# Saro00/DGN

Measured on AMD Instinct MI355X. Metric: dgn_layer_fwd_bwd_edges_per_sec, higher is better.
Workload: dtype f32; 1 GPU; c2: ZINC-12k (12000 molecules, one batch), DGN towers: 5 towers, hidden 70, mean max min dir1-av dir1-dx x identity amplification attenuation; edges_per_gpu=586426, nodes_per_gpu=275167, parallelism=single GPU, step=edge weights + layer forward + backward

## Files before the change

dgn_amd/csrc/dgn_abi.hip:

```cpp
#include <hip/hip_runtime.h>

#include <atomic>
#include <cstdarg>
#include <cstdio>
#include <cstdlib>
#include <cstring>
#include <mutex>

#include "dgn_common.hpp"

namespace dgn {
namespace {
thread_local char g_err[512] = "";
}

void set_error(const char* fmt, ...) {
    va_list ap;
    va_start(ap, fmt);
    vsnprintf(g_err, sizeof(g_err), fmt, ap);
    va_end(ap);
}

namespace {
__global__ void zero_rows_kernel(int64_t rows, int64_t width, int64_t ld, float* __restrict__ p) {
// ... 68 lines not shown
    {"tile_gemm", "DGN_TILE_GEMM", -1, false},
    {"tile_wgrad", "DGN_TILE_WGRAD", -1, false},
    {"no_zmask", "DGN_NO_ZMASK", 0, true},
    {"linear_small_min_waves", "DGN_LINEAR_SMALL_MIN_WAVES", 8, false},
    {"graph_bwd_tiles", "DGN_GRAPH_BWD_TILES", 0, false},
    {"odd_direct", "DGN_ODD_DIRECT", 1, false},
    {"bn_from_wgrad", "DGN_BN_FROM_WGRAD", 1, false},
    {"mix_bwd_fused", "DGN_MIX_BWD_FUSED", 1, false},
    {"blk_lds_pad_kb", "DGN_BLK_LDS_PAD_KB", 0, false},
    {"lin_wreg", "DGN_LIN_WREG", 3, false},
    {"bd_bwd_fused", "DGN_BD_BWD_FUSED", 1, false},
    {"bn_stats_fused", "DGN_BN_STATS_FUSED", 1, false},
    {"ew_big_min", "DGN_EW_BIG_MIN", 1 << 19, false},
    {"ew_separate", "DGN_EW_SEPARATE", 0, true},
    {"ew_no_flat8", "DGN_EW_NO_FLAT8", 0, true},
};
std::atomic<int64_t> g_opt[OPT_COUNT];
std::once_flag g_opt_once;
void init_options() {
    for (int i = 0; i < OPT_COUNT; ++i) {
        const char* e = getenv(kOpts[i].env);
        g_opt[i].store(e ? (kOpts[i].presence ? 1 : atoll(e)) : kOpts[i].def, std::memory_order_relaxed);
    }
    if (getenv("DGN_NO_MIX_FUSED")) g_opt[OPT_NO_ZMASK].store(1, std::memory_order_relaxed);
}
int find_option(const char* name) {
    if (name)
        for (int i = 0; i < OPT_COUNT; ++i)
            if (!strcmp(name, kOpts[i].name)) return i;
    return -1;
// ... 32 lines not shown
```

dgn_amd/csrc/dgn_agg.hip:

```cpp
#include <hip/hip_runtime.h>

#include <algorithm>
#include <cstdlib>

#include "dgn_agg_kernels.hpp"

namespace dgn {
namespace {

bool aligned(const void* ptr, int bytes) { return (reinterpret_cast<uintptr_t>(ptr) % bytes) == 0; }

int pick_vec(const DgnAggSpec* spec, const DgnMsg* msg, const float* out, int64_t ld_out, const DgnMsgGrad* gr) {
    const int64_t Ft = msg->F / spec->n_towers;
    for (int vec : {4, 2}) {
        if (msg->f_valid && vec != 2) continue;
        bool ok = (msg->F % vec == 0) && (Ft % vec == 0) && (ld_out % vec == 0) && aligned(out, 4 * vec) && (spec->tower_stride % vec == 0);
        if (msg->F / vec <= 32 && vec > 2) ok = false;
        auto chk = [&](const float* ptr, int64_t ld) {
            if (ptr && (!aligned(ptr, 4 * vec) || ld % vec != 0)) ok = false;
        };
        if (!msg->f_valid) chk(msg->x_src, msg->ld_src);
        chk(msg->x_dst, msg->ld_dst);
        chk(msg->m_edge, msg->ld_edge);
        if (!msg->f_valid) chk(msg->x_in, msg->ld_in);
// ... 314 lines not shown

extern "C" int dgn_agg_backward_aux(const DgnGraph* g, const DgnAggSpec* spec, const DgnMsg* msg, const float* w, int64_t ld_w,
                                    const float* log_deg, const float* g_out, int64_t ld_gout, const unsigned char* aux,
                                    const DgnMsgGrad* grads, void* ws, size_t ws_bytes, void* stream_) {
    if (g && g->n_nodes == 0 && spec && msg && grads) return validate(g, spec, msg, w, log_deg);
    AggParams p;
    float* tab_part = nullptr;
    int rc = agg_backward_prepare(p, g, spec, msg, w, ld_w, log_deg, g_out, ld_gout, false, grads, ws, ws_bytes, stream_, &tab_part, aux);
    if (rc) return rc;
    hipStream_t stream = static_cast<hipStream_t>(stream_);
    const int vec = pick_vec(spec, msg, g_out, ld_gout, grads);
    const unsigned tiles = (unsigned)((msg->F + kWave * vec - 1) / (kWave * vec));
    if (g->blk_cut && g->blk_gap > 0 && g->n_edges > 0 && grads->accumulate == 0 && g->n_hub == 0 && tiles == 1 && vec == 2 && !msg->edge_type &&
        !msg->m_edge && p.g_src && p.x_src && p.n_src == p.n_nodes && !p.g_edge) {
        p.blk_cut = g->blk_cut;
        const int brc = launch_agg_block_v2(p, g->blk_gap, stream);
        if (brc != 1) return brc;
        p.blk_cut = nullptr;
    }
    if (g->gblk_desc && g->n_gblk > 0 && g->csc_order && g->dst_csr && g->csc_ptr && g->n_edges > 0 && grads->accumulate == 0 && g->n_hub == 0 &&
        tiles == 1 && vec == 2 && !msg->edge_type && !msg->m_edge && p.g_src && p.x_src && p.n_src == p.n_nodes && !p.g_edge && !short_rows(p)) {
        p.gblk_desc = g->gblk_desc; p.n_gblk = (int32_t)g->n_gblk; p.gblk_rows = g->gblk_rows; p.csc_order = g->csc_order; p.dst_csr = g->dst_csr;
        p.csc_ptr = g->csc_ptr;
        const int grc = launch_agg_graph_v2(p, stream);
        if (grc != 1) return grc;
        p.gblk_desc = nullptr;
    }
    rc = launch(vec, p, tiles, stream, true);
    if (rc || !msg->edge_type || !grads->g_edge) return rc;
    const int K = msg->n_edge_types, KF = K * (int)msg->F;
    const int waves = std::max(1, std::min(16, 16384 / KF));
    hipLaunchKernelGGL(edge_table_grad_partial, dim3(kTabBlocks), dim3(kWave * waves), (size_t)waves * KF * sizeof(float), stream,
                       p.stage, p.csc_pos, msg->edge_type, p.n_edges, (int)msg->F, K, tab_part);
// ... 6 lines not shown
```

dgn_amd/csrc/dgn_agg_blk_v2.hip:

```cpp
#include "dgn_agg_block.hpp"
#include "dgn_agg_graph.hpp"

namespace dgn {
int launch_agg_block_v2(const AggParams& p, int gap, hipStream_t stream) { return launch_block_vec<2>(p, gap, stream); }
int launch_agg_graph_v2(const AggParams& p, hipStream_t stream) { return launch_graph_v2(p, stream); }
}
```

dgn_amd/csrc/dgn_agg_block.hpp:

```cpp
#pragma once
#include "dgn_agg_kernels.hpp"

namespace dgn {

constexpr int kBlkRowsMax = 56;

template <class C, class O, bool AUX>
__global__ __launch_bounds__(kWave) void agg_bwd_block(const AggParams p0) {
    extern __shared__ float blk_acc[];
    constexpr int VEC = C::VEC, RB = kBwdShortRows;
    static_assert(RB == 4, "groups of four rows");
    const int64_t n_bins = (p0.n_nodes + p0.blk_bin - 1) / p0.blk_bin;
    const int64_t b = xcd_remap(blockIdx.x, n_bins);
    if (b < 0) return;
    const int N = (int)p0.n_nodes;
    const int lo = p0.blk_cut[b * p0.blk_bin];
    const int hi = p0.blk_cut[min((b + 1) * (int64_t)p0.blk_bin, p0.n_nodes)];
    if (lo >= hi) return;
    AggParams p = p0;
    p.blk_lds = blk_acc; p.blk_lo = lo; p.blk_hi = hi;
    const int lo4 = lo & ~(RB - 1), hi4 = min(N, (hi + RB - 1) & ~(RB - 1));
    const int n_ptr = hi4 - lo4 + 1;
    const int ipv_all = p.indptr[lo4 + min(lane_id(), n_ptr - 1)];
    const int n4 = ((hi - lo) * p.F + 3) >> 2;
    for (int i = lane_id(); i < n4; i += kWave) reinterpret_cast<float4*>(blk_acc)[i] = make_float4(0.f, 0.f, 0.f, 0.f);
    const int f0 = lane_id() * VEC;
    const bool active = f0 < p.F;
    auto ptr_at = [&](int i) { return bcast_i(ipv_all, min(i, n_ptr - 1)); };
    constexpr bool AHEAD = n_gout_blocks<O>() <= 2;
    SlotBatch<C::NCH, C::NW> cur, nxt;
    GroupRows<C, RB, n_gout_blocks<O>(), AUX> rows, rows_nxt;
    cur.load_raw(p, ptr_at(0));
    if constexpr (AHEAD) load_group_rows<C, O, RB, AUX>(rows, p, lo4, f0);
    for (int row0 = lo4; row0 < hi; row0 += RB) {
        const int off = row0 - lo4;
        nxt.load_raw(p, ptr_at(off + RB));
        if constexpr (AHEAD) load_group_rows<C, O, RB, AUX>(rows_nxt, p, row0 + RB, f0);
        const int nrows = min(RB, N - row0);
        const int ipv = __shfl(ipv_all, min(off + min(lane_id(), RB), n_ptr - 1), kWave);
        bwd_short_group<C, O, RB, false, false, AUX, true, AHEAD>(p, row0, nrows, f0, active, ipv, &cur, &rows);
        cur = nxt;
        if constexpr (AHEAD) rows = rows_nxt;
    }
    if (active) {
        for (int r = 0; r < hi - lo; ++r) {
            float v[VEC];
            ldv<VEC>(v, blk_acc + r * p.F + f0);
            stv<VEC>(p.g_src + (int64_t)(lo + r) * p.ldg_src + f0, v);
        }
// ... 7 lines not shown
    const int bin = rcap - gap + 1;
    if (bin < 4) return false;
    out.bin = bin; out.rows = rcap;
    out.lds = (((size_t)rcap * F * 4) + 15) & ~(size_t)15;
    return true;
}

template <class C, class O>
int launch_backward_block_cfg(const AggParams& p, int gap, hipStream_t stream) {
    BlkPlan plan;
    if (p.n_nodes < option(OPT_BLK_MIN_NODES) || !short_rows(p) || option(OPT_BWD_ROWS_PER_WAVE) <= 1 || !blk_plan(plan, p.F, gap)) return 1;
    AggParams q = p;
    q.stage = nullptr; q.csc_pos = nullptr; q.csc_ptr = nullptr; q.fresh = true; q.seg_add = false;
    q.blk_bin = plan.bin; q.blk_rows = plan.rows;
    const int64_t n_bins = (p.n_nodes + plan.bin - 1) / plan.bin;
    const dim3 grid((unsigned)xcd_grid(n_bins)), block(kWave);
    plan.lds += (size_t)std::max<int64_t>(0, option(OPT_BLK_LDS_PAD_KB)) * 1024;
    if constexpr (C::NCH <= 2) {
        if (p.aux) {
            hipLaunchKernelGGL((agg_bwd_block<C, O, true>), grid, block, plan.lds, stream, q);
            DGN_HIP_CHECK(hipGetLastError());
            return DGN_OK;
        }
    }
    hipLaunchKernelGGL((agg_bwd_block<C, O, false>), grid, block, plan.lds, stream, q);
    DGN_HIP_CHECK(hipGetLastError());
    return DGN_OK;
}

template <int VEC>
int launch_block_vec(const AggParams& p, int gap, hipStream_t stream) {
// ... 12 lines not shown
```

dgn_amd/csrc/dgn_agg_kernels.hpp:

```cpp
#pragma once
#include <hip/hip_runtime.h>

#include <cmath>
#include <cstdlib>

#include "dgn_common.hpp"

#ifndef DGN_UNROLL
#define DGN_UNROLL 8
#endif

namespace dgn {

enum : uint32_t {
    NEED_SQ = 2u, NEED_MAX = 4u, NEED_MIN = 8u,
    NEED_XIN = 16u,
    NEED_RECOMP = 32u,
    NEED_M_EMIT = 64u,
    NEED_XPASS = 128u
};

struct AggParams {
    const int32_t* indptr;
    const int32_t* src;
// ... 43 lines not shown
    float* part_sw;
    float* coef;
    float* stage;
    unsigned char* aux;
    int32_t aux_rows;
    int32_t stage_out;
    bool fresh;
    bool seg_add;
    const int32_t* csc_ptr;
    const int32_t* csc_pos;
    int32_t n_slots;
    int32_t n_coef;
    const int32_t* blk_cut;
    int32_t blk_bin;
    int32_t blk_rows;
    const int32_t* gblk_desc; const int32_t* csc_order; const int32_t* dst_csr;
    int32_t n_gblk, gblk_rows;
    float* blk_lds;
    int32_t blk_lo, blk_hi;
};

inline void pack_agg_list(AggParams& p, const DgnAggSpec* spec) {
    p.op_pack = p.ch_pack = 0; p.any_av = false;
    uint32_t need = 0;
    for (int a = 0; a < spec->n_agg; ++a) {
        const int op = spec->agg_op[a], c = spec->agg_ch[a];
        p.op_pack |= (uint64_t)op << (4 * a);
        p.ch_pack |= (uint64_t)((op >= DGN_AGG_DIR_AV && op <= DGN_AGG_DIR_DX_NO_ABS) ? c : 0) << (3 * a);
        switch (op) {
            case DGN_AGG_MAX: need |= NEED_MAX | NEED_RECOMP; break;
// ... 1940 lines not shown
```

dgn_amd/csrc/dgn_common.hpp:

```cpp
#pragma once
#include <hip/hip_runtime.h>
#include <stdint.h>

#include <atomic>

#include "dgn_hip.h"

namespace dgn {

constexpr int kWave = 64;
#ifndef DGN_WAVES_PER_BLOCK
#define DGN_WAVES_PER_BLOCK 1
#endif
constexpr int kWavesPerBlock = DGN_WAVES_PER_BLOCK;
constexpr int kBlock = kWave * kWavesPerBlock;
constexpr int kXcds = 8;

void set_error(const char* fmt, ...);
enum Opt { OPT_BLK_LDS_KB, OPT_BLK_MIN_NODES, OPT_BWD_ROWS_PER_WAVE, OPT_TILE_GEMM, OPT_TILE_WGRAD, OPT_NO_ZMASK, OPT_LINEAR_SMALL_MIN_WAVES, OPT_GRAPH_BWD_TILES, OPT_ODD_DIRECT, OPT_BN_FROM_WGRAD, OPT_MIX_BWD_FUSED, OPT_BLK_LDS_PAD_KB, OPT_LIN_WREG, OPT_BD_BWD_FUSED, OPT_BN_STATS_FUSED, OPT_EW_BIG_MIN, OPT_EW_SEPARATE, OPT_EW_NO_FLAT8, OPT_COUNT };
int64_t option(Opt o);
int hip_fail(hipError_t e, const char* what);
int zero_rows_async(float* p, int64_t rows, int64_t width, int64_t ld, hipStream_t stream);
int scale_rows_async(int64_t n_rows, int32_t width, const float* g, int64_t ld_g, const float* g_loss, float* out, int64_t ld_out, hipStream_t stream);

using LdsOptIn = std::atomic<unsigned long long>;
hipError_t allow_lds(LdsOptIn& done, int bytes, const void* const* kernels, int n_kernels);
template <class... K>
inline hipError_t allow_lds(LdsOptIn& done, int bytes, K*... kernels) {
    const void* const list[] = {reinterpret_cast<const void*>(kernels)...};
    return allow_lds(done, bytes, list, (int)sizeof...(K));
}
int n_cus();
inline bool al16(const void* q) { return (reinterpret_cast<uintptr_t>(q) & 15) == 0; }

// ... 55 lines not shown
__device__ __forceinline__ float bcast_f(float v, int lane) {
    return __int_as_float(__builtin_amdgcn_readlane(__float_as_int(v), lane));
}
__device__ __forceinline__ int uniform_i(int v) { return __builtin_amdgcn_readfirstlane(v); }

__device__ __forceinline__ int64_t xcd_remap(int64_t b, int64_t n_logical) {
#ifdef DGN_EXP_NOREMAP
    return b < n_logical ? b : -1;
#endif
    int64_t per = (n_logical + kXcds - 1) / kXcds;
    int64_t logical = (b % kXcds) * per + b / kXcds;
    return logical < n_logical ? logical : -1;
}
inline int64_t xcd_grid(int64_t n_logical) { return ((n_logical + kXcds - 1) / kXcds) * kXcds; }

template <int VEC>
__device__ __forceinline__ void ldv(float (&d)[VEC], const float* p) {
    if constexpr (VEC == 4) {
        float4 t = *reinterpret_cast<const float4*>(p);
        d[0] = t.x; d[1] = t.y; d[2] = t.z; d[3] = t.w;
    } else if constexpr (VEC == 2) {
        float2 t = *reinterpret_cast<const float2*>(p);
        d[0] = t.x; d[1] = t.y;
    } else {
        d[0] = *p;
    }
}
template <int VEC>
__device__ __forceinline__ void stv(float* p, const float (&d)[VEC]) {
    if constexpr (VEC == 4) {
// ... 86 lines not shown
```

dgn_amd/csrc/dgn_graph_build.hip:

```cpp
#include <hip/hip_runtime.h>
#include <hipcub/hipcub.hpp>

#include <cmath>
#include <cstdint>

#include "dgn_common.hpp"

namespace dgn {
namespace {

inline size_t up256(size_t x) { return (x + 255) & ~(size_t)255; }
inline unsigned blocks(int64_t n, int per = 256) { return (unsigned)((n + per - 1) / per); }
inline int bits_for(int64_t n) { int b = 1; while (((int64_t)1 << b) < n && b < 31) ++b; return b; }

__global__ void gb_prepare(int64_t E, const int64_t* __restrict__ dst, int32_t* __restrict__ key, int32_t* __restrict__ val,
                           int32_t* __restrict__ deg) {
    const int64_t e = (int64_t)blockIdx.x * blockDim.x + threadIdx.x;
    if (e >= E) return;
    const int d = (int)dst[e];
    key[e] = d;
    val[e] = (int)e;
    atomicAdd(deg + d, 1);
}
__global__ void gb_gather(int64_t E, const int64_t* __restrict__ src, const int32_t* __restrict__ perm, int32_t* __restrict__ src_csr,
// ... 39 lines not shown
        atomicAdd(diff + a + 1, 1);
        atomicAdd(diff + b + 1, -1);
    }
}
__global__ void gb_mark_closed(int64_t N, const int32_t* __restrict__ cross, int32_t* __restrict__ val) {
    const int64_t i = (int64_t)blockIdx.x * blockDim.x + threadIdx.x;
    if (i <= N) val[i] = cross[i] == 0 ? (int)i : 0;
}
__global__ void gb_max_gap(int64_t N, const int32_t* __restrict__ cross, const int32_t* __restrict__ lastcut, int32_t* __restrict__ gap_out) {
    const int64_t i = (int64_t)blockIdx.x * blockDim.x + threadIdx.x + 1;
    int g = 0;
    if (i <= N && cross[i] == 0) g = (int)i - lastcut[i - 1];
#pragma unroll
    for (int o = 32; o > 0; o >>= 1) g = max(g, __shfl_xor(g, o, kWave));
    if ((threadIdx.x & 63) == 0 && g > 0) atomicMax(gap_out, g);
}

size_t cub_bytes(int64_t n) {
    size_t a = 0, b = 0;
    int32_t* p = nullptr;
    hipcub::DeviceRadixSort::SortPairs(nullptr, a, p, p, p, p, (int)n);
    hipcub::DeviceScan::ExclusiveSum(nullptr, b, p, p, (int)n);
    size_t c = 0;
    hipcub::DeviceScan::InclusiveScan(nullptr, c, p, p, hipcub::Max(), (int)n);
    return up256(std::max(std::max(a, b), c)) + 256;
}

}
}

// ... 49 lines not shown
    int32_t* cross = reinterpret_cast<int32_t*>(w); w += nbytes;
    int32_t* val = reinterpret_cast<int32_t*>(w); w += nbytes;
    void* cub = w;
    size_t cub_sz = ws_bytes - (size_t)(w - static_cast<char*>(ws));
    DGN_HIP_CHECK(hipMemsetAsync(diff, 0, (size_t)(n_nodes + 2) * 4, st));
    DGN_HIP_CHECK(hipMemsetAsync(gap_out, 0, sizeof(int32_t), st));
    if (n_edges > 0) hipLaunchKernelGGL(gb_span, dim3(blocks(n_edges)), dim3(256), 0, st, n_edges, src_csr, dst_csr, diff);
    DGN_HIP_CHECK(hipcub::DeviceScan::InclusiveSum(cub, cub_sz, diff, cross, (int)(n_nodes + 1), st));
    hipLaunchKernelGGL(gb_mark_closed, dim3(blocks(n_nodes + 1)), dim3(256), 0, st, n_nodes, cross, val);
    DGN_HIP_CHECK(hipcub::DeviceScan::InclusiveScan(cub, cub_sz, val, blk_cut, hipcub::Max(), (int)(n_nodes + 1), st));
    if (n_nodes > 0) hipLaunchKernelGGL(gb_max_gap, dim3(blocks(n_nodes)), dim3(256), 0, st, n_nodes, cross, blk_cut, gap_out);
    DGN_HIP_CHECK(hipGetLastError());
    return DGN_OK;
}

extern "C" int dgn_graph_build_csc(int64_t n_nodes, int64_t n_edges, const int32_t* src_csr, int32_t* csc_ptr, int32_t* csc_pos,
                                   int32_t* csc_order, void* ws, size_t ws_bytes, void* stream_) {
    const char* fn = "dgn_graph_build_csc";
    if (!csc_ptr || (n_edges > 0 && (!src_csr || !csc_pos || !csc_order))) { set_error("%s: null array", fn); return DGN_ERR_INVALID; }
    if (!ws || ws_bytes < dgn_graph_build_workspace_bytes(n_nodes, n_edges)) { set_error("%s: workspace too small", fn); return DGN_ERR_WORKSPACE; }
    hipStream_t st = static_cast<hipStream_t>(stream_);
    char* w = static_cast<char*>(ws);
    const size_t eb = up256((size_t)(n_edges + 1) * 4), nbytes = up256((size_t)(n_nodes + 2) * 4);
    int32_t* val = reinterpret_cast<int32_t*>(w); w += eb;
    int32_t* key_out = reinterpret_cast<int32_t*>(w); w += eb;
    w += 2 * eb;
    int32_t* hist = reinterpret_cast<int32_t*>(w); w += nbytes;
    w += 3 * nbytes;
    w += up256((size_t)n_edges + 1);
    void* cub = w;
// ... 12 lines not shown
```

dgn_amd/graph.py:

```python
from __future__ import annotations

import ctypes as C
import os
from typing import Dict, Optional, Tuple

import functools

import torch

from . import _lib
from .spec import EPS, AggPlan, Channel

HUB_THRESHOLD = 2048
HUB_CHUNK = 1024
NATIVE_BUILD = True
DC_CLASSES, DC_UNIT = _lib.DGN_DC_CLASSES, _lib.DGN_DC_UNIT
GRAPH_BLOCK_MAX_ROWS = 512
BLOCK_MAX_GAP = 52
DEFERRED_STATS = True


def _ptr(t: Optional[torch.Tensor]) -> Optional[int]:
    return None if t is None else t.data_ptr()

# ... 141 lines not shown
                ent["overflow_event"].record(torch.cuda.current_stream(self.device))
                ent["overflow_pending"] = True
                self._check_block_overflow(ent)
        if not getattr(self, "_stats_pending", False):
            return
        self._stats_event.synchronize()
        self._stats_pending = False
        max_deg, n_hub = int(self._stats_host[0]), int(self._stats_host[1])
        self.max_in_degree = max_deg
        if n_hub:
            raise _lib.DgnError("padded graphs take batches without hub rows (in-degree <= hub_threshold) only "
                                f"(the batch loaded before this call had {n_hub}, largest in-degree {max_deg})")

    def invalidate_caches(self) -> None:
        self._wcache.clear()
        for k in ("_scale_cache", "_dst_slots", "_eig_norm", "_slot_types", "_dc", "_dc_split", "_dc_scale", "_blk", "_blk_tables"):
            self.__dict__.pop(k, None)
        if hasattr(self, "_c"):
            self._c.blk_cut, self._c.blk_gap = None, 0
            self._c.gblk_desc, self._c.n_gblk, self._c.gblk_rows, self._c.dst_csr = None, 0, 0, None

    def _build_native(self, src, dst, num_nodes, hub_threshold, hub_chunk):
        lib = _lib.load()
        dev, E = src.device, src.numel()
        if num_nodes >= 2 ** 31 - 1 or E >= 2 ** 31 - 1:
            raise ValueError("graph exceeds the int32 CSR range")
        src64, dst64 = src.long().contiguous(), dst.long().contiguous()
        i32 = lambda n: torch.empty(n, dtype=torch.int32, device=dev)
        indptr, src_csr, dst_csr = i32(num_nodes + 1), i32(E), i32(E)
        eid = torch.empty(E, dtype=torch.int64, device=dev)
        log_deg = torch.empty(num_nodes, dtype=torch.float32, device=dev)
        deg = torch.empty(num_nodes, dtype=torch.int64, device=dev)
        stats = i32(4)
        nbytes = lib.dgn_graph_build_workspace_bytes(num_nodes, E)
# ... 133 lines not shown
        self.csc_ptr, self.csc_pos, order = i32(N + 1), i32(E), i32(E)
        self.csc_order = order
        _lib.check(lib.dgn_graph_build_csc(N, E, self.src.data_ptr(), self.csc_ptr.data_ptr(), self.csc_pos.data_ptr(), order.data_ptr(),
                                           ws.data_ptr(), nbytes, stream), "dgn_graph_build_csc")
        self._c.csc_ptr, self._c.csc_pos = self.csc_ptr.data_ptr(), self.csc_pos.data_ptr()

    def _closed_cuts(self):
        if "_blk" not in self.__dict__:
            lib = _lib.load()
            N, E, dev = self.num_nodes, self.num_edges, self.device
            dst_csr = getattr(self, "dst_csr", None)
            if dst_csr is None:
                deg = (self.indptr[1:] - self.indptr[:-1]).long()
                dst_csr = torch.repeat_interleave(torch.arange(N, device=dev, dtype=torch.int32), deg)
                self.dst_csr = dst_csr
            cut = torch.empty(N + 1, dtype=torch.int32, device=dev)
            gap = torch.zeros(1, dtype=torch.int32, device=dev)
            nbytes = lib.dgn_graph_build_workspace_bytes(N, E)
            ws = torch.empty(nbytes, dtype=torch.uint8, device=dev)
            _lib.check(lib.dgn_graph_build_cuts(N, E, self.src.data_ptr(), dst_csr.data_ptr(), cut.data_ptr(), gap.data_ptr(),
                                                ws.data_ptr(), nbytes, _lib.stream_ptr(dev)), "dgn_graph_build_cuts")
            self._blk = (cut, int(gap.item()))
        return self._blk

    def block_table(self, graph_sizes=None, target_rows=None):
        if getattr(self, "_pad", None) is not None:
            return self.__dict__.get("_blk_static") if target_rows is None else None
        tables = self.__dict__.setdefault("_blk_tables", {})
        ent = tables.get(target_rows)
        if ent is not None:
            return ent or None
        if not (self.src.is_cuda and self.num_src == self.num_nodes and self.n_hub == 0 and getattr(self, "_pad", None) is None
                and self.row_base == 0 and self.num_edges > 0 and self.num_nodes > 0):
            tables[target_rows] = {}
            return None
        if torch.cuda.is_current_stream_capturing():
            return None
        import numpy as np
# ... 65 lines not shown
        ent["desc"].copy_(ent["host"], non_blocking=True)
        ent["copied"].record(torch.cuda.current_stream(self.device))
        ent["overflow_host"].copy_(ent["overflow"], non_blocking=True)
        ent["overflow_event"].record(torch.cuda.current_stream(self.device))
        ent["overflow_pending"] = True

    def _check_block_overflow(self, ent) -> None:
        if ent.get("overflow_pending"):
            ent["overflow_event"].synchronize()
            ent["overflow_pending"] = False
            if int(ent["overflow_host"][0]):
                ent["overflow"].zero_()
                raise _lib.DgnError(f"a batch held a graph beyond the block capacity ({ent['max_rows']} rows / {ent['max_edges']} edges): its rows "
                                    "were skipped by the graph-block layer kernels (set_block_capacity with larger bounds)")

    def ensure_blocks(self, enabled: bool = True) -> bool:
        ok = False
        min_nodes = int(_lib.options.blk_min_nodes)
        if enabled and self.src.is_cuda and self.num_src == self.num_nodes and self.n_hub == 0 and getattr(self, "_pad", None) is None \
                and self.num_nodes >= max(1, min_nodes) and 0 < self.num_edges <= 3 * self.num_nodes and self.row_base == 0:
            if "_blk" not in self.__dict__ and torch.cuda.is_current_stream_capturing():
                enabled = False
            if enabled and "_blk" not in self.__dict__:
                self._closed_cuts()
            if enabled:
                cut, gap = self._blk
                ok = 0 < gap <= BLOCK_MAX_GAP
        if ok:
            self._c.blk_cut, self._c.blk_gap = cut.data_ptr(), gap
        else:
            self._c.blk_cut, self._c.blk_gap = None, 0
        self._ensure_graph_blocks(enabled)
        return ok

    def _ensure_graph_blocks(self, enabled: bool = True) -> bool:
        ok = False
        if enabled and self.src.is_cuda and self.num_src == self.num_nodes and self.n_hub == 0 and getattr(self, "_pad", None) is None \
                and self.row_base == 0 and self.num_edges > 3 * self.num_nodes:
            t = self.block_table(target_rows=1)
            if t is not None and t["max_rows"] <= GRAPH_BLOCK_MAX_ROWS and getattr(self, "_csc_ready", False) and hasattr(self, "csc_order"):
                self._closed_cuts()
                self._c.gblk_desc, self._c.n_gblk, self._c.gblk_rows = t["desc"].data_ptr(), t["n_blocks"], t["max_rows"]
                self._c.csc_order, self._c.dst_csr = self.csc_order.data_ptr(), self.dst_csr.data_ptr()
                ok = True
        if not ok:
            self._c.gblk_desc, self._c.n_gblk, self._c.gblk_rows, self._c.csc_order, self._c.dst_csr = None, 0, 0, None, None
# ... 93 lines not shown
```

dgn_amd/ops.py:

```python
from __future__ import annotations

import ctypes as C
import os
from typing import Optional

import torch

from . import _lib
from .graph import DGNGraph, _ptr
from .spec import EPS, AggPlan


DETERMINISTIC_BACKWARD = "auto"


def _two_phase_scatter(F: int) -> bool:
    return (F % 2 == 0) if DETERMINISTIC_BACKWARD == "auto" else bool(DETERMINISTIC_BACKWARD)


BLOCK_BACKWARD = os.environ.get("DGN_BLOCK_BACKWARD", "1") != "0"

_N_VALID = None


# ... 121 lines not shown
    grads.g_src, grads.ld_src = _ptr(g_src), _ld(g_src)
    grads.g_dst, grads.ld_dst = _ptr(g_dst), _ld(g_dst)
    grads.g_edge, grads.ld_edge = _ptr(g_edge), _ld(g_edge)
    grads.g_in, grads.ld_in = _ptr(g_in), _ld(g_in)
    msg = _msg_struct(F, x_src, x_dst, m_edge, x_in, edge_type, f_valid)
    stream = _lib.stream_ptr(dev)
    tower_stride, ld_gout = _out_layout(g_out)
    specs = _spec_structs(plan, n_towers, avg_log, tower_stride)
    g = graph.c_graph
    first = True
    deterministic = _two_phase_scatter(F) and g_src is not None
    if edge_type is not None and not deterministic:
        raise _lib.DgnError("edge-type table: the backward needs the two-phase scatter (even F, a gradient for x_src)")
    if deterministic:
        graph.ensure_csc()
    graph.ensure_blocks(bool(BLOCK_BACKWARD) and deterministic and not accumulate and len(plan.launches) == 1)
    for spec, l in zip(specs, plan.launches):
        nbytes = lib.dgn_agg_backward_workspace_bytes(C.byref(g), C.byref(spec), F, 1 if deterministic else 0)
        if edge_type is not None:
            nbytes += lib.dgn_agg_edge_table_workspace_bytes(F, m_edge.shape[0])
        ws = torch.empty(nbytes, dtype=torch.uint8, device=dev) if nbytes else None
        wl = w[l.ch_offset:] if (w is not None and l.channels) else None
        tmp = None
        if g_edge is not None and not first:
            tmp = torch.empty_like(g_edge)
            grads.g_edge = tmp.data_ptr()
        grads.accumulate = 1 if (accumulate or not first) else 0
        rc = lib.dgn_agg_backward_aux(C.byref(g), C.byref(spec), C.byref(msg), _ptr(wl), w.stride(0) if w is not None else 0,
                                      graph.log_deg.data_ptr(), g_out.data_ptr(), ld_gout, _ptr(aux), C.byref(grads),
                                      _ptr(ws), nbytes, stream)
        _lib.check(rc, "dgn_agg_backward")
# ... 804 lines not shown
        return out

    @staticmethod
    def backward(ctx, g_out):
        lib = _lib.load()
        w_edge, h, snorm, scale, w_sd, bias_sd, w_post, b_post, gamma, beta, w_mix, b_mix, saved_buf, aux, drop_mask = ctx.saved_tensors
        graph, plan, cfg = ctx.graph, ctx.plan, ctx.cfg
        T, fi, fo, S = cfg[:4]
        id_slot = cfg[9] if len(cfg) > 9 else None
        N, Fm, Fo = h.shape[0], T * fi, T * fo
        K = plan.n_agg * fi
        dev = h.device
        _, bufs = _carve(_towers_saved_sizes(cfg, plan, N, ctx.n_y1, ctx.n_z), dev, saved_buf)
        g_out = g_out.contiguous()
        graph.ensure_csc()
        graph.ensure_blocks(bool(BLOCK_BACKWARD))
        L, keep = _towers_struct(graph, plan, ctx.avg_log, w_edge, cfg, h, snorm, scale, w_sd, bias_sd, w_post, b_post, gamma, beta, w_mix, b_mix, bufs,
                                 ctx.use_mask, aux, drop_mask, ctx.n_valid)
        L.id_slot1 = 0 if id_slot is None else int(id_slot) + 1
        ws = _layer_workspace(L, lib.dgn_towers_layer_backward_workspace_bytes(C.byref(L)), dev)
        g_h = torch.empty((N, Fm), dtype=torch.float32, device=dev)
        n_ops = [2 * Fm * Fm, 2 * Fm, Fo, Fo, Fo, T * S * fo * K]
        n_flat = _up64(sum(n_ops))
        gbuf = torch.empty(n_flat + _up64(Fo * Fo) + Fo, dtype=torch.float32, device=dev)
        g_w_sd, g_bias_sd, g_b_post, g_gamma, g_beta, g_w_post = gbuf[:sum(n_ops)].split(n_ops)
        g_w_mix, g_b_mix = gbuf[n_flat:n_flat + Fo * Fo], gbuf[n_flat + _up64(Fo * Fo):]
        G = _lib.DgnTowersGrads(g_out=g_out.data_ptr(), g_h=g_h.data_ptr(), g_w_sd=g_w_sd.data_ptr(), g_bias_sd=g_bias_sd.data_ptr(),
                                g_w_post=g_w_post.data_ptr(), g_b_post=g_b_post.data_ptr(), g_gamma=g_gamma.data_ptr(),
                                g_beta=g_beta.data_ptr(), g_w_mix=g_w_mix.data_ptr(), g_b_mix=g_b_mix.data_ptr())
        _lib.check(lib.dgn_towers_layer_backward(C.byref(L), C.byref(G), _lib.stream_ptr(dev)), "dgn_towers_layer_backward")
        return (None, None, None, None, None, g_h, None, None, None, None, None, g_w_sd.view(2 * Fm, Fm), g_bias_sd, g_w_post.view(T, S * fo, K),
# ... 242 lines not shown
        ctx.save_for_backward(w_edge, h, snorm, scale, w_pre, b_pre, w_post, b_post, gamma, beta, saved_buf, aux)
        ctx.graph, ctx.plan, ctx.avg_log, ctx.cfg = graph, plan, avg_log, cfg
        return out

    @staticmethod
    def backward(ctx, g_out):
        lib = _lib.load()
        w_edge, h, snorm, scale, w_pre, b_pre, w_post, b_post, gamma, beta, saved_buf, aux = ctx.saved_tensors
        cfg, graph = ctx.cfg, ctx.graph
        type_net, F0, fo = cfg[:3]
        N, dev = h.shape[0], h.device
        sizes, Fp, K = _dense_sizes(cfg, N, ctx.dc is not None)
        _, bufs = _carve_ptrs(sizes, dev, saved_buf)
        g_out = g_out.contiguous()
        graph.ensure_csc()
        graph.ensure_blocks(bool(BLOCK_BACKWARD))
        L, keep = _dense_struct(graph, ctx.plan, ctx.avg_log, w_edge, cfg, h, snorm, scale, w_pre, b_pre, w_post, b_post, gamma, beta, bufs, ctx.n_valid,
                                ctx.dc)
        L.agg_aux = _ptr(aux)
        ws = _layer_workspace(L, lib.dgn_dense_layer_backward_workspace_bytes(C.byref(L)), dev)
        g_h = torch.empty((N, F0), dtype=torch.float32, device=dev)
        n_pre = w_pre.numel() if w_pre is not None else 0
        _, (g_w_pre, g_b_pre, g_w_post, g_b_post, g_gamma, g_beta) = _carve([n_pre, F0 if (type_net == 1 and b_pre is not None) else 0, w_post.numel(), fo, fo, fo], dev)
        q = lambda t: t.data_ptr() if t.numel() else None
        G = _lib.DgnDenseGrads(g_out=g_out.data_ptr(), g_h=g_h.data_ptr(), g_w_pre=q(g_w_pre), g_b_pre=q(g_b_pre), g_w_post=g_w_post.data_ptr(),
                               g_b_post=g_b_post.data_ptr(), g_gamma=g_gamma.data_ptr(), g_beta=g_beta.data_ptr())
        stream = _lib.stream_ptr(dev)
        _lib.check(lib.dgn_dense_layer_backward(C.byref(L), C.byref(G), stream), "dgn_dense_layer_backward")
        return (None, None, None, None, None, g_h, None, None, None, None, None,
                g_w_pre.view_as(w_pre) if w_pre is not None else None, g_b_pre if (b_pre is not None and type_net == 1) else None,
                g_w_post.view_as(w_post), g_b_post if b_post is not None else None, g_gamma, g_beta)
# ... 786 lines not shown
```

include/dgn_hip.h:

```cpp
#ifndef DGN_HIP_H
#define DGN_HIP_H

#include <stddef.h>
#include <stdint.h>

#ifdef __cplusplus
extern "C" {
#endif

#define DGN_ABI_VERSION 38

#define DGN_MAX_AGG 16
#define DGN_MAX_CH 4
#define DGN_MAX_SCALERS 4

enum {
    DGN_OK = 0,
    DGN_ERR_INVALID = -1,
    DGN_ERR_WORKSPACE = -2,
    DGN_ERR_HIP = -3
};

enum {
    DGN_AGG_MEAN = 0,
    DGN_AGG_SUM = 1,
// ... 27 lines not shown
    const int32_t* src;
    int64_t n_hub;
    const int32_t* hub_rows;
    const int32_t* hub_chunk_ptr;
    int64_t n_chunks;
    const int32_t* chunk_hub;
    int32_t hub_threshold;
    int32_t hub_chunk;
    const int32_t* csc_ptr;
    const int32_t* csc_pos;
    int32_t max_in_degree;
    int64_t n_src;
    int64_t row_base;
    const int32_t* blk_cut;
    int32_t blk_gap;
    const int32_t* gblk_desc; int64_t n_gblk; int32_t gblk_rows;
    const int32_t* csc_order;
    const int32_t* dst_csr;
} DgnGraph;

typedef struct DgnChannel {
    int32_t kind;
    int32_t eig_col;
    float alpha;
    float eps;
} DgnChannel;

typedef struct DgnAggSpec {
    int32_t n_agg;
    int32_t agg_op[DGN_MAX_AGG];
// ... 163 lines not shown
                   int64_t lddw, float* dbias, void* ws, size_t ws_bytes, void* stream);

int dgn_layer_fused_supported(const DgnGraph* g, const DgnAggSpec* spec, int64_t F, int32_t n_scalers, int32_t f_out);
int dgn_layer_fused_forward(const DgnGraph* g, const DgnAggSpec* spec, const DgnMsg* msg, const float* w, int64_t ld_w,
                            const float* log_deg, const float* weight, int64_t ldw, int64_t stride_w, int32_t n_scalers,
                            int32_t f_out, const float* scale, const float* bias, const float* row_scale, float* y, int64_t ld_y,
                            void* stream);
size_t dgn_graph_build_workspace_bytes(int64_t n_nodes, int64_t n_edges);
int dgn_graph_build(int64_t n_nodes, int64_t n_edges, const int64_t* src, const int64_t* dst, int32_t* indptr, int32_t* src_csr,
                    int32_t* dst_csr, int64_t* eid, float* log_deg, int64_t* in_degree, int32_t* stats, int32_t hub_threshold,
                    void* ws, size_t ws_bytes, void* stream);
int dgn_graph_build_cuts(int64_t n_nodes, int64_t n_edges, const int32_t* src_csr, const int32_t* dst_csr, int32_t* blk_cut,
                         int32_t* gap_out, void* ws, size_t ws_bytes, void* stream);
int dgn_graph_build_csc(int64_t n_nodes, int64_t n_edges, const int32_t* src_csr, int32_t* csc_ptr, int32_t* csc_pos,
                        int32_t* csc_order, void* ws, size_t ws_bytes, void* stream);


typedef struct DgnTowersLayer {
    const DgnGraph* graph;
    const DgnAggSpec* spec;
    const float* w;
    int64_t ld_w;
    const float* log_deg;
    int32_t n_towers, f_in, f_out, n_scalers;
    int32_t residual;
    float momentum, eps, slope;
    const float* h;
    const float* snorm;
    const float* scale;
    const float* w_sd;  const float* bias_sd;
// ... 281 lines not shown
```

Baseline: 506.8 million edges/s.

## Schedule block-backward bins from a precomputed, work-sorted task list

Adds a per-graph task list of int4 records (row range, starting edge pointer, group count), built once after the block cuts, and sorts the bins by descending work so heavy bins launch first. The block backward kernel reads its task from this list instead of the XCD remap and cut lookups, and in the EARLY case it preloads the first group's rows and the next slot batch before entering the main loop. The intent is to reduce tail imbalance and startup latency per block. In exchange it adds a one-time radix sort and task build stored past the end of the cut array, drops the XCD-aware block mapping, and has extra logic for graph-capture caching.

```diff
diff --git a/dgn_amd/csrc/dgn_abi.hip b/dgn_amd/csrc/dgn_abi.hip
--- a/dgn_amd/csrc/dgn_abi.hip
+++ b/dgn_amd/csrc/dgn_abi.hip
@@ -106,6 +106,7 @@
     {"ew_big_min", "DGN_EW_BIG_MIN", 1 << 19, false},
     {"ew_separate", "DGN_EW_SEPARATE", 0, true},
     {"ew_no_flat8", "DGN_EW_NO_FLAT8", 0, true},
+    {"blk_task_list", "DGN_BLK_TASK_LIST", 2, false},
 };
 std::atomic<int64_t> g_opt[OPT_COUNT];
 std::once_flag g_opt_once;
diff --git a/dgn_amd/csrc/dgn_agg.hip b/dgn_amd/csrc/dgn_agg.hip
--- a/dgn_amd/csrc/dgn_agg.hip
+++ b/dgn_amd/csrc/dgn_agg.hip
@@ -352,9 +352,13 @@
     if (g->blk_cut && g->blk_gap > 0 && g->n_edges > 0 && grads->accumulate == 0 && g->n_hub == 0 && tiles == 1 && vec == 2 && !msg->edge_type &&
         !msg->m_edge && p.g_src && p.x_src && p.n_src == p.n_nodes && !p.g_edge) {
         p.blk_cut = g->blk_cut;
+        if (g->blk_task_bin > 0) {
+            p.blk_task = reinterpret_cast<const int4*>(g->blk_cut + blk_task_offset(g->n_nodes));
+            p.blk_task_bin = g->blk_task_bin;
+        }
         const int brc = launch_agg_block_v2(p, g->blk_gap, stream);
         if (brc != 1) return brc;
-        p.blk_cut = nullptr;
+        p.blk_cut = nullptr; p.blk_task = nullptr; p.blk_task_bin = 0;
     }
     if (g->gblk_desc && g->n_gblk > 0 && g->csc_order && g->dst_csr && g->csc_ptr && g->n_edges > 0 && grads->accumulate == 0 && g->n_hub == 0 &&
         tiles == 1 && vec == 2 && !msg->edge_type && !msg->m_edge && p.g_src && p.x_src && p.n_src == p.n_nodes && !p.g_edge && !short_rows(p)) {
diff --git a/dgn_amd/csrc/dgn_agg_blk_v2.hip b/dgn_amd/csrc/dgn_agg_blk_v2.hip
--- a/dgn_amd/csrc/dgn_agg_blk_v2.hip
+++ b/dgn_amd/csrc/dgn_agg_blk_v2.hip
@@ -5,3 +5,11 @@
 int launch_agg_block_v2(const AggParams& p, int gap, hipStream_t stream) { return launch_block_vec<2>(p, gap, stream); }
 int launch_agg_graph_v2(const AggParams& p, hipStream_t stream) { return launch_graph_v2(p, stream); }
 }
+
+extern "C" int dgn_agg_block_plan(int64_t F, int32_t gap, int32_t* bin, int32_t* rows) {
+    dgn::BlkPlan plan;
+    if (F <= 0 || gap <= 0 || !dgn::blk_plan(plan, F, gap)) return 1;
+    if (bin) *bin = plan.bin;
+    if (rows) *rows = plan.rows;
+    return 0;
+}
diff --git a/dgn_amd/csrc/dgn_agg_block.hpp b/dgn_amd/csrc/dgn_agg_block.hpp
--- a/dgn_amd/csrc/dgn_agg_block.hpp
+++ b/dgn_amd/csrc/dgn_agg_block.hpp
@@ -11,11 +11,19 @@
     constexpr int VEC = C::VEC, RB = kBwdShortRows;
     static_assert(RB == 4, "groups of four rows");
     const int64_t n_bins = (p0.n_nodes + p0.blk_bin - 1) / p0.blk_bin;
-    const int64_t b = xcd_remap(blockIdx.x, n_bins);
-    if (b < 0) return;
     const int N = (int)p0.n_nodes;
-    const int lo = p0.blk_cut[b * p0.blk_bin];
-    const int hi = p0.blk_cut[min((b + 1) * (int64_t)p0.blk_bin, p0.n_nodes)];
+    const bool listed = p0.blk_task != nullptr;
+    int lo, hi, ptr0 = 0;
+    if (listed) {
+        if ((int64_t)blockIdx.x >= n_bins) return;
+        const int4 t = p0.blk_task[blockIdx.x];
+        lo = t.x; hi = t.y; ptr0 = t.z;
+    } else {
+        const int64_t b = xcd_remap(blockIdx.x, n_bins);
+        if (b < 0) return;
+        lo = p0.blk_cut[b * p0.blk_bin];
+        hi = p0.blk_cut[min((b + 1) * (int64_t)p0.blk_bin, p0.n_nodes)];
+    }
     if (lo >= hi) return;
     AggParams p = p0;
     p.blk_lds = blk_acc; p.blk_lo = lo; p.blk_hi = hi;
@@ -30,9 +38,20 @@
     constexpr bool AHEAD = n_gout_blocks<O>() <= 2;
     SlotBatch<C::NCH, C::NW> cur, nxt;
     GroupRows<C, RB, n_gout_blocks<O>(), AUX> rows, rows_nxt;
-    cur.load_raw(p, ptr_at(0));
-    if constexpr (AHEAD) load_group_rows<C, O, RB, AUX>(rows, p, lo4, f0);
-    for (int row0 = lo4; row0 < hi; row0 += RB) {
+    constexpr bool EARLY = !AHEAD && (n_gout_blocks<O>() <= 4 || (n_gout_blocks<O>() == 5 && AUX));
+    cur.load_raw(p, listed ? ptr0 : ptr_at(0));
+    if (AHEAD || (EARLY && listed)) load_group_rows<C, O, RB, AUX>(rows, p, lo4, f0);
+    int row0 = lo4;
+    if constexpr (EARLY) {
+        if (listed) {
+            nxt.load_raw(p, ptr_at(RB));
+            const int ipv = __shfl(ipv_all, min(min(lane_id(), RB), n_ptr - 1), kWave);
+            bwd_short_group<C, O, RB, false, false, AUX, true, true>(p, row0, min(RB, N - row0), f0, active, ipv, &cur, &rows);
+            cur = nxt;
+            row0 += RB;
+        }
+    }
+    for (; row0 < hi; row0 += RB) {
         const int off = row0 - lo4;
         nxt.load_raw(p, ptr_at(off + RB));
         if constexpr (AHEAD) load_group_rows<C, O, RB, AUX>(rows_nxt, p, row0 + RB, f0);
@@ -70,7 +89,8 @@
     q.stage = nullptr; q.csc_pos = nullptr; q.csc_ptr = nullptr; q.fresh = true; q.seg_add = false;
     q.blk_bin = plan.bin; q.blk_rows = plan.rows;
     const int64_t n_bins = (p.n_nodes + plan.bin - 1) / plan.bin;
-    const dim3 grid((unsigned)xcd_grid(n_bins)), block(kWave);
+    if (p.blk_task_bin != plan.bin || option(OPT_BLK_TASK_LIST) == 0) q.blk_task = nullptr;
+    const dim3 grid((unsigned)(q.blk_task ? n_bins : xcd_grid(n_bins))), block(kWave);
     plan.lds += (size_t)std::max<int64_t>(0, option(OPT_BLK_LDS_PAD_KB)) * 1024;
     if constexpr (C::NCH <= 2) {
         if (p.aux) {
diff --git a/dgn_amd/csrc/dgn_agg_kernels.hpp b/dgn_amd/csrc/dgn_agg_kernels.hpp
--- a/dgn_amd/csrc/dgn_agg_kernels.hpp
+++ b/dgn_amd/csrc/dgn_agg_kernels.hpp
@@ -81,6 +81,8 @@
     const int32_t* blk_cut;
     int32_t blk_bin;
     int32_t blk_rows;
+    const int4* blk_task;
+    int32_t blk_task_bin;
     const int32_t* gblk_desc; const int32_t* csc_order; const int32_t* dst_csr;
     int32_t n_gblk, gblk_rows;
     float* blk_lds;
diff --git a/dgn_amd/csrc/dgn_common.hpp b/dgn_amd/csrc/dgn_common.hpp
--- a/dgn_amd/csrc/dgn_common.hpp
+++ b/dgn_amd/csrc/dgn_common.hpp
@@ -17,7 +17,7 @@
 constexpr int kXcds = 8;
 
 void set_error(const char* fmt, ...);
-enum Opt { OPT_BLK_LDS_KB, OPT_BLK_MIN_NODES, OPT_BWD_ROWS_PER_WAVE, OPT_TILE_GEMM, OPT_TILE_WGRAD, OPT_NO_ZMASK, OPT_LINEAR_SMALL_MIN_WAVES, OPT_GRAPH_BWD_TILES, OPT_ODD_DIRECT, OPT_BN_FROM_WGRAD, OPT_MIX_BWD_FUSED, OPT_BLK_LDS_PAD_KB, OPT_LIN_WREG, OPT_BD_BWD_FUSED, OPT_BN_STATS_FUSED, OPT_EW_BIG_MIN, OPT_EW_SEPARATE, OPT_EW_NO_FLAT8, OPT_COUNT };
+enum Opt { OPT_BLK_LDS_KB, OPT_BLK_MIN_NODES, OPT_BWD_ROWS_PER_WAVE, OPT_TILE_GEMM, OPT_TILE_WGRAD, OPT_NO_ZMASK, OPT_LINEAR_SMALL_MIN_WAVES, OPT_GRAPH_BWD_TILES, OPT_ODD_DIRECT, OPT_BN_FROM_WGRAD, OPT_MIX_BWD_FUSED, OPT_BLK_LDS_PAD_KB, OPT_LIN_WREG, OPT_BD_BWD_FUSED, OPT_BN_STATS_FUSED, OPT_EW_BIG_MIN, OPT_EW_SEPARATE, OPT_EW_NO_FLAT8, OPT_BLK_TASK_LIST, OPT_COUNT };
 int64_t option(Opt o);
 int hip_fail(hipError_t e, const char* what);
 int zero_rows_async(float* p, int64_t rows, int64_t width, int64_t ld, hipStream_t stream);
@@ -103,6 +103,8 @@
 }
 inline int64_t xcd_grid(int64_t n_logical) { return ((n_logical + kXcds - 1) / kXcds) * kXcds; }
 
+inline int64_t blk_task_offset(int64_t n_nodes) { return (n_nodes + 4) & ~(int64_t)3; }
+
 template <int VEC>
 __device__ __forceinline__ void ldv(float (&d)[VEC], const float* p) {
     if constexpr (VEC == 4) {
diff --git a/dgn_amd/csrc/dgn_graph_build.hip b/dgn_amd/csrc/dgn_graph_build.hip
--- a/dgn_amd/csrc/dgn_graph_build.hip
+++ b/dgn_amd/csrc/dgn_graph_build.hip
@@ -77,6 +77,31 @@
 #pragma unroll
     for (int o = 32; o > 0; o >>= 1) g = max(g, __shfl_xor(g, o, kWave));
     if ((threadIdx.x & 63) == 0 && g > 0) atomicMax(gap_out, g);
+}
+
+__device__ __forceinline__ int4 gb_task_of(int64_t b, int64_t N, int bin, const int32_t* __restrict__ cut, const int32_t* __restrict__ indptr) {
+    const int lo = cut[b * bin], hi = cut[min((b + 1) * (int64_t)bin, N)];
+    if (lo >= hi) return make_int4(lo, hi, indptr[lo & ~3], 0);
+    return make_int4(lo, hi, indptr[lo & ~3], (hi - (lo & ~3) + 3) >> 2);
+}
+constexpr int kTaskKeyBits = 5;
+__global__ void gb_task_keys(int64_t n_bins, int64_t N, int bin, const int32_t* __restrict__ cut, const int32_t* __restrict__ indptr,
+                             int32_t* __restrict__ key, int32_t* __restrict__ val) {
+    const int64_t b = (int64_t)blockIdx.x * blockDim.x + threadIdx.x;
+    if (b >= n_bins) return;
+    key[b] = min(gb_task_of(b, N, bin, cut, indptr).w, (1 << kTaskKeyBits) - 1);
+    val[b] = (int)b;
+}
+__global__ void gb_task_records(int64_t n_bins, int64_t N, int bin, const int32_t* __restrict__ cut, const int32_t* __restrict__ indptr,
+                                const int32_t* __restrict__ order, int4* __restrict__ tasks) {
+    const int64_t i = (int64_t)blockIdx.x * blockDim.x + threadIdx.x;
+    if (i < n_bins) tasks[i] = gb_task_of(order ? order[i] : i, N, bin, cut, indptr);
+}
+size_t task_sort_bytes(int64_t n) {
+    size_t a = 0;
+    int32_t* p = nullptr;
+    hipcub::DeviceRadixSort::SortPairsDescending(nullptr, a, p, p, p, p, (int)n, 0, kTaskKeyBits);
+    return up256(a) + 256;
 }
 
 size_t cub_bytes(int64_t n) {
@@ -156,6 +181,46 @@
     return DGN_OK;
 }
 
+extern "C" int64_t dgn_blk_cut_capacity(int64_t n_nodes) {
+    return n_nodes < 0 ? 0 : blk_task_offset(n_nodes) + 4 * ((n_nodes + 3) / 4);
+}
+
+extern "C" size_t dgn_graph_build_tasks_workspace_bytes(int64_t n_nodes, int32_t bin) {
+    if (n_nodes < 0 || bin < 4) return 0;
+    const int64_t n_bins = (n_nodes + bin - 1) / bin;
+    return 4 * up256((size_t)(n_bins + 1) * 4) + task_sort_bytes(n_bins + 1);
+}
+
+extern "C" int dgn_graph_build_tasks(int64_t n_nodes, const int32_t* indptr, int32_t* blk_cut, int32_t bin, void* ws, size_t ws_bytes,
+                                     void* stream_) {
+    const char* fn = "dgn_graph_build_tasks";
+    if (n_nodes < 0 || n_nodes >= INT32_MAX - 1) { set_error("%s: sizes outside the int32 CSR range", fn); return DGN_ERR_INVALID; }
+    if (bin < 4) { set_error("%s: a bin has at least 4 rows", fn); return DGN_ERR_INVALID; }
+    if (!blk_cut || !indptr) { set_error("%s: null array", fn); return DGN_ERR_INVALID; }
+    if (reinterpret_cast<uintptr_t>(blk_cut) & 15) { set_error("%s: blk_cut is not 16-byte aligned", fn); return DGN_ERR_INVALID; }
+    if (!ws || ws_bytes < dgn_graph_build_tasks_workspace_bytes(n_nodes, bin)) { set_error("%s: workspace too small", fn); return DGN_ERR_WORKSPACE; }
+    if (n_nodes == 0) return DGN_OK;
+    hipStream_t st = static_cast<hipStream_t>(stream_);
+    const int64_t n_bins = (n_nodes + bin - 1) / bin;
+    int4* tasks = reinterpret_cast<int4*>(blk_cut + blk_task_offset(n_nodes));
+    const int32_t* order = nullptr;
+    if (option(OPT_BLK_TASK_LIST) != 1) {
+        char* w = static_cast<char*>(ws);
+        const size_t kb = up256((size_t)(n_bins + 1) * 4);
+        int32_t* key = reinterpret_cast<int32_t*>(w); w += kb;
+        int32_t* key_out = reinterpret_cast<int32_t*>(w); w += kb;
+        int32_t* val = reinterpret_cast<int32_t*>(w); w += kb;
+        int32_t* val_out = reinterpret_cast<int32_t*>(w); w += kb;
+        size_t cub_sz = ws_bytes - (size_t)(w - static_cast<char*>(ws));
+        hipLaunchKernelGGL(gb_task_keys, dim3(blocks(n_bins)), dim3(256), 0, st, n_bins, n_nodes, (int)bin, (const int32_t*)blk_cut, indptr, key, val);
+        DGN_HIP_CHECK(hipcub::DeviceRadixSort::SortPairsDescending(w, cub_sz, key, key_out, val, val_out, (int)n_bins, 0, kTaskKeyBits, st));
+        order = val_out;
+    }
+    hipLaunchKernelGGL(gb_task_records, dim3(blocks(n_bins)), dim3(256), 0, st, n_bins, n_nodes, (int)bin, (const int32_t*)blk_cut, indptr, order, tasks);
+    DGN_HIP_CHECK(hipGetLastError());
+    return DGN_OK;
+}
+
 extern "C" int dgn_graph_build_csc(int64_t n_nodes, int64_t n_edges, const int32_t* src_csr, int32_t* csc_ptr, int32_t* csc_pos,
                                    int32_t* csc_order, void* ws, size_t ws_bytes, void* stream_) {
     const char* fn = "dgn_graph_build_csc";
diff --git a/dgn_amd/graph.py b/dgn_amd/graph.py
--- a/dgn_amd/graph.py
+++ b/dgn_amd/graph.py
@@ -179,10 +179,10 @@
 
     def invalidate_caches(self) -> None:
         self._wcache.clear()
-        for k in ("_scale_cache", "_dst_slots", "_eig_norm", "_slot_types", "_dc", "_dc_split", "_dc_scale", "_blk", "_blk_tables"):
+        for k in ("_scale_cache", "_dst_slots", "_eig_norm", "_slot_types", "_dc", "_dc_split", "_dc_scale", "_blk", "_blk_tasks", "_blk_tasks_captured", "_blk_tables"):
             self.__dict__.pop(k, None)
         if hasattr(self, "_c"):
-            self._c.blk_cut, self._c.blk_gap = None, 0
+            self._c.blk_cut, self._c.blk_gap, self._c.blk_task_bin = None, 0, 0
             self._c.gblk_desc, self._c.n_gblk, self._c.gblk_rows, self._c.dst_csr = None, 0, 0, None
 
     def _build_native(self, src, dst, num_nodes, hub_threshold, hub_chunk):
@@ -346,14 +346,39 @@
                 deg = (self.indptr[1:] - self.indptr[:-1]).long()
                 dst_csr = torch.repeat_interleave(torch.arange(N, device=dev, dtype=torch.int32), deg)
                 self.dst_csr = dst_csr
-            cut = torch.empty(N + 1, dtype=torch.int32, device=dev)
+            cut = torch.empty(lib.dgn_blk_cut_capacity(N), dtype=torch.int32, device=dev)[:N + 1]
             gap = torch.zeros(1, dtype=torch.int32, device=dev)
             nbytes = lib.dgn_graph_build_workspace_bytes(N, E)
             ws = torch.empty(nbytes, dtype=torch.uint8, device=dev)
             _lib.check(lib.dgn_graph_build_cuts(N, E, self.src.data_ptr(), dst_csr.data_ptr(), cut.data_ptr(), gap.data_ptr(),
                                                 ws.data_ptr(), nbytes, _lib.stream_ptr(dev)), "dgn_graph_build_cuts")
             self._blk = (cut, int(gap.item()))
+            self.__dict__.pop("_blk_tasks", None)
+            self.__dict__.pop("_blk_tasks_captured", None)
         return self._blk
+
+    def _block_tasks(self, width: int) -> int:
+        lib = _lib.load()
+        mode = int(_lib.options.blk_task_list)
+        cut, gap = self._blk
+        bin_ = C.c_int32(0)
+        if mode == 0 or lib.dgn_agg_block_plan(int(width), gap, C.byref(bin_), None) != 0:
+            return 0
+        key = (bin_.value, mode)
+        capturing = torch.cuda.is_current_stream_capturing()
+        if self.__dict__.get("_blk_tasks") != key:
+            if capturing or self.__dict__.get("_blk_tasks_captured"):
+                return 0
+            N, dev = self.num_nodes, self.device
+            nbytes = lib.dgn_graph_build_tasks_workspace_bytes(N, bin_.value)
+            ws = torch.empty(nbytes, dtype=torch.uint8, device=dev)
+            self.__dict__.pop("_blk_tasks", None)
+            _lib.check(lib.dgn_graph_build_tasks(N, self.indptr.data_ptr(), cut.data_ptr(), bin_.value, ws.data_ptr(), nbytes,
+                                                 _lib.stream_ptr(dev)), "dgn_graph_build_tasks")
+            self._blk_tasks = key
+        if capturing:
+            self._blk_tasks_captured = True
+        return bin_.value
 
     def block_table(self, graph_sizes=None, target_rows=None):
         if getattr(self, "_pad", None) is not None:
@@ -449,7 +474,7 @@
                 raise _lib.DgnError(f"a batch held a graph beyond the block capacity ({ent['max_rows']} rows / {ent['max_edges']} edges): its rows "
                                     "were skipped by the graph-block layer kernels (set_block_capacity with larger bounds)")
 
-    def ensure_blocks(self, enabled: bool = True) -> bool:
+    def ensure_blocks(self, enabled: bool = True, width: int = 0) -> bool:
         ok = False
         min_nodes = int(_lib.options.blk_min_nodes)
         if enabled and self.src.is_cuda and self.num_src == self.num_nodes and self.n_hub == 0 and getattr(self, "_pad", None) is None \
@@ -463,8 +488,9 @@
                 ok = 0 < gap <= BLOCK_MAX_GAP
         if ok:
             self._c.blk_cut, self._c.blk_gap = cut.data_ptr(), gap
+            self._c.blk_task_bin = self._block_tasks(width) if width > 0 else 0
         else:
-            self._c.blk_cut, self._c.blk_gap = None, 0
+            self._c.blk_cut, self._c.blk_gap, self._c.blk_task_bin = None, 0, 0
         self._ensure_graph_blocks(enabled)
         return ok
 
diff --git a/dgn_amd/ops.py b/dgn_amd/ops.py
--- a/dgn_amd/ops.py
+++ b/dgn_amd/ops.py
@@ -159,7 +159,7 @@
         raise _lib.DgnError("edge-type table: the backward needs the two-phase scatter (even F, a gradient for x_src)")
     if deterministic:
         graph.ensure_csc()
-    graph.ensure_blocks(bool(BLOCK_BACKWARD) and deterministic and not accumulate and len(plan.launches) == 1)
+    graph.ensure_blocks(bool(BLOCK_BACKWARD) and deterministic and not accumulate and len(plan.launches) == 1, F)
     for spec, l in zip(specs, plan.launches):
         nbytes = lib.dgn_agg_backward_workspace_bytes(C.byref(g), C.byref(spec), F, 1 if deterministic else 0)
         if edge_type is not None:
@@ -994,7 +994,7 @@
         _, bufs = _carve(_towers_saved_sizes(cfg, plan, N, ctx.n_y1, ctx.n_z), dev, saved_buf)
         g_out = g_out.contiguous()
         graph.ensure_csc()
-        graph.ensure_blocks(bool(BLOCK_BACKWARD))
+        graph.ensure_blocks(bool(BLOCK_BACKWARD), Fm)
         L, keep = _towers_struct(graph, plan, ctx.avg_log, w_edge, cfg, h, snorm, scale, w_sd, bias_sd, w_post, b_post, gamma, beta, w_mix, b_mix, bufs,
                                  ctx.use_mask, aux, drop_mask, ctx.n_valid)
         L.id_slot1 = 0 if id_slot is None else int(id_slot) + 1
@@ -1267,7 +1267,7 @@
         _, bufs = _carve_ptrs(sizes, dev, saved_buf)
         g_out = g_out.contiguous()
         graph.ensure_csc()
-        graph.ensure_blocks(bool(BLOCK_BACKWARD))
+        graph.ensure_blocks(bool(BLOCK_BACKWARD), Fp)
         L, keep = _dense_struct(graph, ctx.plan, ctx.avg_log, w_edge, cfg, h, snorm, scale, w_pre, b_pre, w_post, b_post, gamma, beta, bufs, ctx.n_valid,
                                 ctx.dc)
         L.agg_aux = _ptr(aux)
diff --git a/include/dgn_hip.h b/include/dgn_hip.h
--- a/include/dgn_hip.h
+++ b/include/dgn_hip.h
@@ -8,7 +8,7 @@
 extern "C" {
 #endif
 
-#define DGN_ABI_VERSION 38
+#define DGN_ABI_VERSION 39
 
 #define DGN_MAX_AGG 16
 #define DGN_MAX_CH 4
@@ -66,6 +66,7 @@
     int64_t row_base;
     const int32_t* blk_cut;
     int32_t blk_gap;
+    int32_t blk_task_bin;
     const int32_t* gblk_desc; int64_t n_gblk; int32_t gblk_rows;
     const int32_t* csc_order;
     const int32_t* dst_csr;
@@ -259,6 +260,11 @@
                          int32_t* gap_out, void* ws, size_t ws_bytes, void* stream);
 int dgn_graph_build_csc(int64_t n_nodes, int64_t n_edges, const int32_t* src_csr, int32_t* csc_ptr, int32_t* csc_pos,
                         int32_t* csc_order, void* ws, size_t ws_bytes, void* stream);
+int dgn_agg_block_plan(int64_t F, int32_t gap, int32_t* bin, int32_t* rows);
+int64_t dgn_blk_cut_capacity(int64_t n_nodes);
+size_t dgn_graph_build_tasks_workspace_bytes(int64_t n_nodes, int32_t bin);
+int dgn_graph_build_tasks(int64_t n_nodes, const int32_t* indptr, int32_t* blk_cut, int32_t bin, void* ws, size_t ws_bytes,
+                          void* stream);
 
 
 typedef struct DgnTowersLayer {
```

New measurement: 502.8 million edges/s. About the same (-0.8%).
